# scverse/scanpy

Measured on AMD Instinct MI355X. Metric: cells/sec through pca+neighbors+leiden, 1M x 2k CSR, higher is better.
Workload: dtype bf16x3

## Files before the change

### scanpy_amd/_kernels.py

```python
from __future__ import annotations

import ctypes as C

import torch

from . import _lib
from ._device import ptr, require_gpu, stream_ptr, workspace_pool

import os as _os

_POISON = _os.environ.get("SCAMD_POISON_WORKSPACE") == "1"
_GUARD = _os.environ.get("SCAMD_GUARD") == "1"
_GUARD_BYTES = 4096
_CANARY = 0xC5
_guards: list = []


def _guarded(nbytes: int, dev: torch.device, label: str) -> torch.Tensor:
    pay = (int(nbytes) + 255) // 256 * 256
    raw = torch.empty(pay + 2 * _GUARD_BYTES, dtype=torch.uint8, device=dev)
    raw[:_GUARD_BYTES] = _CANARY
    raw[_GUARD_BYTES + int(nbytes):] = _CANARY
    _guards.append((label, raw, int(nbytes)))
    return raw[_GUARD_BYTES:_GUARD_BYTES + int(nbytes)]
# ... 232 lines not shown
    dev = require_gpu()
    lib = _lib.load()
    gp = (g + 127) // 128 * 128
    gram = _empty((gp, gp), dtype=torch.int64, device=dev)
    colsum = _empty(gp, dtype=torch.int64, device=dev)
    ws, wsz = _ws(lib.scamd_csr_gram_workspace_bytes(n, g), dev)
    rc = lib.scamd_csr_gram_f32(ptr(indptr), ptr(indices), ptr(data), n, g, data.numel(), int(scale_bits), ptr(gram),
                                gp, ptr(colsum), None, ptr(ws), wsz, stream_ptr())
    _check(rc, "scamd_csr_gram_f32")
    return gram, colsum


def spmm(indptr, indices, data, n: int, g: int, b: torch.Tensor, shift: torch.Tensor | None = None) -> torch.Tensor:
    dev = require_gpu()
    b = b.to(torch.float32).contiguous()
    assert b.shape[0] == g
    l = b.shape[1]
    y = _empty((n, l), dtype=torch.float32, device=dev)
    if shift is not None:
        shift = shift.to(torch.float32).contiguous()
    _check(_lib.load().scamd_spmm_csr_f32(ptr(indptr), ptr(indices), ptr(data), n, g, ptr(b), l, ptr(shift),
                                              ptr(y), stream_ptr()), "scamd_spmm_csr_f32")
    return y


def spmm_f64acc(indptr, indices, data, n_rows: int, b: torch.Tensor, scale: torch.Tensor | None = None,
                colsum: torch.Tensor | None = None) -> torch.Tensor:
    dev = require_gpu()
    lib = _lib.load()
    assert b.dtype == torch.float32 and b.is_contiguous()
    l = b.shape[1]
    nnz = data.numel()
    w = _empty((n_rows, l), dtype=torch.float64, device=dev)
    ws, wsz = _ws(lib.scamd_spmm_f64acc_workspace_bytes(n_rows, nnz, l), dev)
    rc = lib.scamd_spmm_csr_f32_f64acc(ptr(indptr), ptr(indices), ptr(data), n_rows, nnz, ptr(b), l, ptr(scale),
                                       ptr(colsum), ptr(w), ptr(ws), wsz, stream_ptr())
    _check(rc, "scamd_spmm_csr_f32_f64acc")
    return w


def dense_debug(op: int, in0: torch.Tensor, in1: torch.Tensor | None = None):
    dev = require_gpu()
    lib = _lib.load()
    in0 = in0.to(torch.float64).contiguous()
    flag = C.c_int(0)
    if op == 1:
        in1 = in1.to(torch.float64).contiguous()
        kdim, m = in0.shape
        n = in1.shape[1]
        out = _empty((m, n), dtype=torch.float64, device=dev)
        rc = lib.scamd_dense_debug_f64(1, ptr(in0), ptr(in1), m, n, kdim, ptr(out), None, C.byref(flag), stream_ptr())
        _check(rc, "scamd_dense_debug_f64")
        return out
    m = in0.shape[0]
    out0 = _empty((m, m) if op == 2 else (m,), dtype=torch.float64, device=dev)
    out1 = _empty((m, m), dtype=torch.float64, device=dev)
    rc = lib.scamd_dense_debug_f64(op, ptr(in0), None, m, m, m, ptr(out0), ptr(out1), C.byref(flag), stream_ptr())
    _check(rc, "scamd_dense_debug_f64")
    return (out0, int(flag.value)) if op == 2 else (out0, out1, int(flag.value))


def eigh_topk(a: torch.Tensor, k: int, *, seed: int = 0, tol: float = 2e-8):
    dev = require_gpu()
    lib = _lib.load()
    assert a.dtype == torch.float64 and a.dim() == 2 and a.shape[0] == a.shape[1] and a.is_cuda
    a = a.contiguous()
    g = a.shape[0]
    lam = _empty(k, dtype=torch.float64, device=dev)
    v = _empty((g, k), dtype=torch.float64, device=dev)
    info = (C.c_int32 * 12)()
    need = lib.scamd_eigh_topk_workspace_bytes(g, k)
    ws, wsz = _ws(need, dev)
    rc = lib.scamd_eigh_topk_f64(ptr(a), g, a.stride(0), k, int(seed) & (2**64 - 1), float(tol), ptr(lam), ptr(v), info,
                                 ptr(ws), wsz, stream_ptr())
    _check(rc, "scamd_eigh_topk_f64")
    resid = C.cast(C.byref(info, 16), C.POINTER(C.c_double))[0]
    return lam, v, {"n_outer": info[0], "n_gemm": info[1], "block_size": info[2], "chol_retries": info[3], "residual": resid}


def pca_csr(indptr, indices, data, n: int, g: int, n_comps: int, *, zero_center: bool = True, seed: int = 0,
            tol: float = 2e-8):
    dev = require_gpu()
    lib = _lib.load()
    k = int(n_comps)
    scores = _empty((n, k), dtype=torch.float32, device=dev)
    comps = _empty((k, g), dtype=torch.float64, device=dev)
    var = _empty(k, dtype=torch.float64, device=dev)
    ratio = _empty(k, dtype=torch.float64, device=dev)
    mean = _empty(g, dtype=torch.float64, device=dev)
    info = (C.c_int32 * 12)()
    need = lib.scamd_pca_csr_workspace_bytes(n, g, k)
    ws, wsz = _ws(need, dev)
    rc = lib.scamd_pca_csr_f32(ptr(indptr), ptr(indices), ptr(data), n, g, data.numel(), k, 1 if zero_center else 0,
                               int(seed) & (2**64 - 1), float(tol), ptr(scores), ptr(comps), ptr(var), ptr(ratio), ptr(mean),
                               info, ptr(ws), wsz, stream_ptr())
    _check(rc, "scamd_pca_csr_f32")
    resid = C.cast(C.byref(info, 16), C.POINTER(C.c_double))[0]
    return scores, comps, var, ratio, mean, {"n_outer": info[0], "n_gemm": info[1], "block_size": info[2],
                                             "chol_retries": info[3], "residual": resid, "scale_bits": info[6]}


def pca_solve_gram(gram_q: torch.Tensor, colsum_q: torch.Tensor, n_total: int, g: int, scale_bits: int, n_comps: int, *,
                   zero_center: bool = True, seed: int = 0, tol: float = 2e-8):
    dev = require_gpu()
    lib = _lib.load()
    k = int(n_comps)
# ... 249 lines not shown
```

### scanpy_amd/csrc/dense.hip

```cpp
#include "common.h"

#include <algorithm>
#include <cmath>
#include <cstdlib>
#include <vector>

namespace scamd {

using f64x4 = __attribute__((ext_vector_type(4))) double;

constexpr int DB_MAX = 128;
constexpr int DB_LD = DB_MAX + 2;
constexpr int DENSE_BATCH_HOST = DB_MAX - 32;

__device__ __forceinline__ unsigned int dhash32(unsigned int x) {
  x ^= x >> 16;
  x *= 0x7feb352dU;
  x ^= x >> 15;
  x *= 0x846ca68bU;
  x ^= x >> 16;
  return x;
}

template <int CTRL>
__device__ __forceinline__ double dpp_f64(double x) {
  const long long b = __double_as_longlong(x);
  const int lo = __builtin_amdgcn_update_dpp(0, (int)(b & 0xffffffffll), CTRL, 0xf, 0xf, false);
  const int hi = __builtin_amdgcn_update_dpp(0, (int)(b >> 32), CTRL, 0xf, 0xf, false);
  return __longlong_as_double(((long long)hi << 32) | (unsigned int)lo);
}
__device__ __forceinline__ double row16_sum(double x) {
  x += dpp_f64<0x128>(x);
  x += dpp_f64<0x124>(x);
  x += dpp_f64<0x122>(x);
  x += dpp_f64<0x121>(x);
  return x;
}
__device__ __forceinline__ double oct_sum(double x) {
  x += dpp_f64<0xB1>(x);
  x += dpp_f64<0x4E>(x);
  x += dpp_f64<0x141>(x);
  return x;
}

__global__ __launch_bounds__(512) void dgemm_tn_kernel(const double* __restrict__ P, int64_t ldp,
                                                       const double* __restrict__ Q, int64_t ldq, int M, int N, int K,
                                                       double alpha, const double* __restrict__ D1, int64_t ldd1,
                                                       double beta1, const double* __restrict__ D2, int64_t ldd2,
                                                       double beta2, double* __restrict__ C, int64_t ldc) {
  __shared__ double red[8][32 * 32];
  const int lane = threadIdx.x & 63, wave = threadIdx.x >> 6;
  const int l15 = lane & 15, kq = lane >> 4;
  const int m0 = blockIdx.x * 32, n0 = blockIdx.y * 32;
  const int kc = ((K + 7) / 8 + 3) / 4 * 4;
  const int kb = wave * kc, ke = min(K, kb + kc);
  f64x4 acc[2][2];
#pragma unroll
  for (int a = 0; a < 2; ++a)
#pragma unroll
    for (int b = 0; b < 2; ++b)
#pragma unroll
      for (int v = 0; v < 4; ++v) acc[a][b][v] = 0.0;
  const bool mv0 = m0 + l15 < M, mv1 = m0 + 16 + l15 < M;
  const bool nv0 = n0 + l15 < N, nv1 = n0 + 16 + l15 < N;
  const double* pp = P + m0 + l15;
  const double* qq = Q + n0 + l15;
#pragma unroll 4
  for (int k0 = kb; k0 < ke; k0 += 4) {
    const int kk = k0 + kq;
    const bool kv = kk < ke;
    const double a0 = (kv && mv0) ? pp[(int64_t)kk * ldp] : 0.0;
    const double a1 = (kv && mv1) ? pp[(int64_t)kk * ldp + 16] : 0.0;
    const double b0 = (kv && nv0) ? qq[(int64_t)kk * ldq] : 0.0;
    const double b1 = (kv && nv1) ? qq[(int64_t)kk * ldq + 16] : 0.0;
    acc[0][0] = __builtin_amdgcn_mfma_f64_16x16x4f64(a0, b0, acc[0][0], 0, 0, 0);
    acc[0][1] = __builtin_amdgcn_mfma_f64_16x16x4f64(a0, b1, acc[0][1], 0, 0, 0);
    acc[1][0] = __builtin_amdgcn_mfma_f64_16x16x4f64(a1, b0, acc[1][0], 0, 0, 0);
    acc[1][1] = __builtin_amdgcn_mfma_f64_16x16x4f64(a1, b1, acc[1][1], 0, 0, 0);
  }
#pragma unroll
  for (int a = 0; a < 2; ++a)
#pragma unroll
    for (int b = 0; b < 2; ++b)
#pragma unroll
      for (int v = 0; v < 4; ++v) red[wave][(16 * a + kq + 4 * v) * 32 + 16 * b + l15] = acc[a][b][v];
  __syncthreads();
#pragma unroll
  for (int j = 0; j < 2; ++j) {
    const int idx = threadIdx.x + 512 * j;
    const int r = idx >> 5, c = idx & 31;
    const int m = m0 + r, n = n0 + c;
    if (m < M && n < N) {
      double s = (((red[0][idx] + red[1][idx]) + (red[2][idx] + red[3][idx])) +
                  ((red[4][idx] + red[5][idx]) + (red[6][idx] + red[7][idx])));
      s *= alpha;
      if (D1) s += beta1 * D1[(int64_t)m * ldd1 + n];
      if (D2) s += beta2 * D2[(int64_t)m * ldd2 + n];
      C[(int64_t)m * ldc + n] = s;
    }
  }
}

static int dgemm_tn(hipStream_t s, const double* P, int64_t ldp, const double* Q, int64_t ldq, int M, int N, int K,
                    double alpha, const double* D1, int64_t ldd1, double beta1, const double* D2, int64_t ldd2,
                    double beta2, double* C, int64_t ldc) {
  hipLaunchKernelGGL(dgemm_tn_kernel, dim3((M + 31) / 32, (N + 31) / 32), dim3(512), 0, s, P, ldp, Q, ldq, M, N, K,
                     alpha, D1, ldd1, beta1, D2, ldd2, beta2, C, ldc);
  SCAMD_LAUNCH_CHECK();
  return SCAMD_OK;
}

__global__ __launch_bounds__(1024) void chol_factor_kernel(const double* __restrict__ G, int b, double shift,
                                                           double* __restrict__ S, int* __restrict__ flag) {
  extern __shared__ __attribute__((aligned(16))) double sm[];
  double* L = sm;
  double* dinv = sm + DB_MAX * DB_LD;
  const int tid = threadIdx.x;
  const int row = tid >> 3, part = tid & 7;
  for (int j = tid; j < b; j += 1024) {
    const double d = G[(int64_t)j * b + j];
    dinv[j] = d > 0.0 ? 1.0 / sqrt(d) : 0.0;
  }
  __syncthreads();
  for (int e = tid; e < b * b; e += 1024) {
    const int i = e / b, j = e - i * b;
    double v = G[(int64_t)i * b + j] * dinv[i] * dinv[j];
    if (i == j) v = (dinv[i] > 0.0 ? 1.0 : 0.0) + shift;
    L[i * DB_LD + j] = v;
  }
  __syncthreads();
  bool bad = false;
  __shared__ double sh_piv[2];
  for (int j = 0; j < b; ++j) {
    double acc = 0.0;
    const bool mine = row >= j && row < b;
    if (mine)
      for (int k = part; k < j; k += 8) acc = fma(L[row * DB_LD + k], L[j * DB_LD + k], acc);
    acc = oct_sum(acc);
    const double v = mine ? L[row * DB_LD + j] - acc : 0.0;
    if (row == j && part == 0) sh_piv[j & 1] = v;
    __syncthreads();
    const double piv = sh_piv[j & 1];
    if (!(piv > 0.0)) {
      bad = true;
      break;
    }
    if (mine && part == 0) L[row * DB_LD + j] = (row == j) ? sqrt(piv) : v / sqrt(piv);
    __syncthreads();
  }
  if (tid == 0) *flag = bad ? 1 : 0;
  if (bad) return;
  {
    const int c = row;
    const double xcc = c < b ? 1.0 / L[c * DB_LD + c] : 0.0;
    for (int j = 1; j < b; ++j) {
      double acc = 0.0;
      if (c < j) {
        for (int k = c + 1 + part; k < j; k += 8) acc = fma(L[j * DB_LD + k], L[c * DB_LD + k], acc);
        if (part == 0) acc = fma(L[j * DB_LD + c], xcc, acc);
      }
      acc = oct_sum(acc);
      if (c < j && part == 0) L[c * DB_LD + j] = -acc / L[j * DB_LD + j];
      __syncthreads();
    }
  }
  for (int e = tid; e < b * b; e += 1024) {
    const int k = e / b, n = e - k * b;
    double v = 0.0;
    if (n == k) v = 1.0 / L[k * DB_LD + k];
    else if (n > k) v = L[k * DB_LD + n];
    S[e] = v * dinv[k];
  }
}

__global__ __launch_bounds__(256) void panel_small_kernel(const double* __restrict__ Z, const double* __restrict__ S, int g,
                                                          int b, int bo , double* __restrict__ C) {
  __shared__ double zrow[8][DB_MAX];
  const int r = threadIdx.x >> 5, cq = threadIdx.x & 31;
  const int m = blockIdx.x * 8 + r;
  for (int k = cq; k < b; k += 32) zrow[r][k] = (m < g) ? Z[(int64_t)m * b + k] : 0.0;
  __syncthreads();
  if (m >= g) return;
  for (int n0 = cq * 4; n0 < bo; n0 += 128) {
    double c0 = 0.0, c1 = 0.0, c2 = 0.0, c3 = 0.0;
    for (int k = 0; k < b; ++k) {
      const double z = zrow[r][k];
      const double* sp = S + (int64_t)k * bo + n0;
      c0 = fma(z, sp[0], c0);
      if (n0 + 1 < bo) c1 = fma(z, sp[1], c1);
      if (n0 + 2 < bo) c2 = fma(z, sp[2], c2);
      if (n0 + 3 < bo) c3 = fma(z, sp[3], c3);
    }
    double* cp = C + (int64_t)m * bo + n0;
    cp[0] = c0;
    if (n0 + 1 < bo) cp[1] = c1;
    if (n0 + 2 < bo) cp[2] = c2;
    if (n0 + 3 < bo) cp[3] = c3;
  }
}

__global__ __launch_bounds__(512) void jacobi_eigh_kernel(const double* __restrict__ T, int b, double* __restrict__ theta,
                                                          double* __restrict__ Y, int* __restrict__ sweeps_out) {
  extern __shared__ __attribute__((aligned(16))) double sm[];
  double* W = sm;
  double* nrm = sm + DB_MAX * DB_LD;
  __shared__ float off_arr[64];
  __shared__ int rank_of[DB_MAX];
  const int tid = threadIdx.x;
  const int n2 = (b + 1) & ~1;
  for (int e = tid; e < n2 * DB_LD; e += 512) {
    const int c = e / DB_LD, i = e - c * DB_LD;
    W[e] = (c < b && i < b) ? T[(int64_t)i * b + c] : 0.0;
  }
  __syncthreads();
  const int grp = tid >> 3, t8 = tid & 7;
  const int nm1 = n2 - 1;
  int sweep = 0;
  for (; sweep < 30; ++sweep) {
    float my_off = 0.f;
    int p = grp == 0 ? nm1 : grp % nm1;
    int q = grp == 0 ? 0 : (nm1 - grp % nm1) % nm1;
    for (int step = 0; step < nm1; ++step) {
      const bool act = grp < n2 / 2 && p < b && q < b;
      if (act) {
        double* wp = W + p * DB_LD;
        double* wq = W + q * DB_LD;
        double a = 0.0, bb = 0.0, c = 0.0;
        for (int i = t8; i < b; i += 8) {
          const double x = wp[i], y = wq[i];
          a = fma(x, x, a);
          bb = fma(y, y, bb);
          c = fma(x, y, c);
        }
        a = oct_sum(a);
        bb = oct_sum(bb);
        c = oct_sum(c);
        const double ab = a * bb;
        if (c * c > 1e-30 * ab) {
          const double d = bb - a, tau = 2.0 * c;
          const double inv_r = rsqrt(fma(d, d, tau * tau));
          const double h = fma(0.5 * fabs(d), inv_r, 0.5);
          const double inv_cs = rsqrt(h);
          const double cs = h * inv_cs;
          const double sn = (d >= 0.0 ? 0.5 : -0.5) * tau * inv_r * inv_cs;
          for (int i = t8; i < b; i += 8) {
            const double x = wp[i], y = wq[i];
            wp[i] = cs * x - sn * y;
            wq[i] = sn * x + cs * y;
          }
          my_off = fmaxf(my_off, (float)(fabs(c) * rsqrt(ab)));
        }
      }
      if (grp != 0) {
        p = p + 1 == nm1 ? 0 : p + 1;
        q = q + 1 == nm1 ? 0 : q + 1;
      } else {
        q = step + 1;
      }
      __syncthreads();
    }
    if (t8 == 0) off_arr[grp] = my_off;
    __syncthreads();
    float off = 0.f;
    for (int i = 0; i < 64; ++i) off = fmaxf(off, off_arr[i]);
    __syncthreads();
    if (off < 1e-8f) {
      ++sweep;
      break;
    }
  }
  if (tid < n2) {
    double a = 0.0;
    for (int i = 0; i < b; ++i) a = fma(W[tid * DB_LD + i], W[tid * DB_LD + i], a);
    nrm[tid] = tid < b ? sqrt(a) : -1.0;
  }
  __syncthreads();
  if (tid < b) {
    int r = 0;
    const double me = nrm[tid];
    for (int j = 0; j < b; ++j) r += (nrm[j] > me || (nrm[j] == me && j < tid)) ? 1 : 0;
    rank_of[tid] = r;
  }
  __syncthreads();
  for (int c = grp; c < b; c += 64) {
    const double nv = nrm[c];
    const double inv = nv > 0.0 ? 1.0 / nv : 0.0;
    const int r = rank_of[c];
    if (t8 == 0) theta[r] = nv;
    for (int i = t8; i < b; i += 8) Y[(int64_t)i * b + r] = W[c * DB_LD + i] * inv;
  }
  if (tid == 0 && sweeps_out) *sweeps_out = sweep;
}

__global__ void randn_kernel(double* __restrict__ z, int64_t count, unsigned int seed) {
  const int64_t i = (int64_t)blockIdx.x * blockDim.x + threadIdx.x;
  if (i >= count) return;
  const unsigned int h1 = dhash32((unsigned int)i * 0x9E3779B1u + seed);
  const unsigned int h2 = dhash32(h1 ^ 0x85EBCA77u ^ (unsigned int)(i >> 32));
  const double u1 = ((double)h1 + 0.5) * (1.0 / 4294967296.0), u2 = ((double)h2 + 0.5) * (1.0 / 4294967296.0);
  z[i] = sqrt(-2.0 * log(u1)) * cos(6.283185307179586 * u2);
}

__global__ void axpby_kernel(int64_t count, double a, const double* __restrict__ x1, double b,
                             const double* __restrict__ x2, double* __restrict__ y) {
  const int64_t i = (int64_t)blockIdx.x * blockDim.x + threadIdx.x;
  if (i < count) y[i] = a * x1[i] + b * x2[i];
}

__global__ void symmetrize_kernel(double* __restrict__ t, int b) {
  const int e = blockIdx.x * blockDim.x + threadIdx.x;
  if (e >= b * b) return;
  const int i = e / b, j = e - i * b;
  if (j > i) {
    const double v = 0.5 * (t[(int64_t)i * b + j] + t[(int64_t)j * b + i]);
    t[(int64_t)i * b + j] = v;
    t[(int64_t)j * b + i] = v;
  }
}

__global__ __launch_bounds__(1024) void rq_minmax_kernel(const double* __restrict__ Z, const double* __restrict__ AZ, int g,
                                                         int b, double* __restrict__ out) {
  __shared__ double part[8][DB_MAX];
  const int c = threadIdx.x & 127, rr = threadIdx.x >> 7;
  double s = 0.0;
  if (c < b) {
    double s1 = 0.0, s2 = 0.0, s3 = 0.0;
    int m = rr;
    for (; m + 24 < g; m += 32) {
      s = fma(Z[(int64_t)m * b + c], AZ[(int64_t)m * b + c], s);
      s1 = fma(Z[(int64_t)(m + 8) * b + c], AZ[(int64_t)(m + 8) * b + c], s1);
      s2 = fma(Z[(int64_t)(m + 16) * b + c], AZ[(int64_t)(m + 16) * b + c], s2);
      s3 = fma(Z[(int64_t)(m + 24) * b + c], AZ[(int64_t)(m + 24) * b + c], s3);
    }
    for (; m < g; m += 8) s = fma(Z[(int64_t)m * b + c], AZ[(int64_t)m * b + c], s);
    s = (s + s1) + (s2 + s3);
  }
  part[rr][c] = s;
  __syncthreads();
  if (threadIdx.x == 0) {
    double mn = INFINITY, mx = -INFINITY;
    for (int j = 0; j < b; ++j) {
      double t = 0.0;
      for (int r = 0; r < 8; ++r) t += part[r][j];
      mn = fmin(mn, t);
      mx = fmax(mx, t);
    }
    out[1] = mn;
    out[2] = mx;
  }
}

__global__ __launch_bounds__(1024) void residual_kernel(const double* __restrict__ V, const double* __restrict__ AV,
                                                        const double* __restrict__ theta, int g, int b, int k,
                                                        double* __restrict__ out) {
  __shared__ double part[8][DB_MAX];
  const int c = threadIdx.x & 127, rr = threadIdx.x >> 7;
  double s = 0.0;
  if (c < k) {
    const double th = theta[c];
    double s1 = 0.0, s2 = 0.0, s3 = 0.0;
    int m = rr;
    for (; m + 24 < g; m += 32) {
      const double d0 = AV[(int64_t)m * b + c] - th * V[(int64_t)m * b + c];
      const double d1 = AV[(int64_t)(m + 8) * b + c] - th * V[(int64_t)(m + 8) * b + c];
      const double d2 = AV[(int64_t)(m + 16) * b + c] - th * V[(int64_t)(m + 16) * b + c];
      const double d3 = AV[(int64_t)(m + 24) * b + c] - th * V[(int64_t)(m + 24) * b + c];
      s = fma(d0, d0, s);
      s1 = fma(d1, d1, s1);
      s2 = fma(d2, d2, s2);
      s3 = fma(d3, d3, s3);
// ... 247 lines not shown
}

}

using namespace scamd;

extern "C" size_t scamd_eigh_topk_workspace_bytes(int64_t g, int k) {
  if (g < 1 || k < 1) return 0;
  Workspace ws(nullptr, 0);
  DenseBuffers d;
  dense_carve(ws, g, dense_block_size(g, k), &d);
  return ws.used();
}

extern "C" int scamd_eigh_topk_f64(const double* a, int64_t g, int64_t lda, int k, uint64_t seed, double tol,
                                   double* lam, double* v, int32_t* info_host, void* workspace, size_t workspace_bytes,
                                   scamd_stream_t stream) {
  SCAMD_REQUIRE(a && lam && v, SCAMD_EINVAL, "eigh_topk: null pointer");
  SCAMD_REQUIRE(g >= 1 && lda >= g && k >= 1 && k <= g, SCAMD_EINVAL, "eigh_topk: bad shape g=%lld k=%d", (long long)g, k);
  SCAMD_REQUIRE(g < ((int64_t)1 << 30), SCAMD_EUNSUPPORTED, "eigh_topk: g too large");
  const int b = dense_block_size(g, k);
  SCAMD_REQUIRE(b == g || k + 32 <= b, SCAMD_EUNSUPPORTED,
                "eigh_topk: k=%d needs a block beyond %d columns (use a full eigendecomposition)", k, DB_MAX);
  SCAMD_REQUIRE(b == g || g >= 2 * b, SCAMD_EUNSUPPORTED, "eigh_topk: g=%lld between %d and %d is served by a full eigh",
                (long long)g, DB_MAX, 2 * DB_MAX);
  DenseOp cx;
  cx.s = stream;
  cx.a = a;
  cx.lda = lda;
  cx.g = (int)g;
  Workspace ws(workspace, workspace_bytes);
  cx.carve(ws, b);
  SCAMD_REQUIRE(workspace && ws.ok, SCAMD_EWORKSPACE, "eigh_topk: workspace %zu < required %zu", workspace_bytes, ws.used());
  DenseStats st;
  int rc = dense_topk(cx, k, eigensolver_seed(seed, 12345u), tol, st);
  if (rc != SCAMD_OK) return rc;
  SCAMD_HIP_CHECK(hipMemcpyAsync(lam, cx.w.theta, sizeof(double) * k, hipMemcpyDeviceToDevice, stream));
  SCAMD_HIP_CHECK(hipMemcpy2DAsync(v, sizeof(double) * k, cx.d.z[3], sizeof(double) * b, sizeof(double) * k, (size_t)g,
                                   hipMemcpyDeviceToDevice, stream));
  SCAMD_HIP_CHECK(hipStreamSynchronize(stream));
  st.n_gemm = cx.n_gemm;
  st.n_chol_retry = cx.n_chol_retry;
  pack_dense_info(info_host, st, -1);
  return SCAMD_OK;
}

extern "C" int scamd_dense_debug_f64(int op, const double* in0, const double* in1, int m, int n, int kdim, double* out0,
                                     double* out1, int32_t* flag_host, scamd_stream_t stream) {
  SCAMD_REQUIRE(in0 && out0, SCAMD_EINVAL, "dense_debug: null pointer");
  if (op == 1) {
    SCAMD_REQUIRE(in1, SCAMD_EINVAL, "dense_debug: null pointer");
    int rc = dgemm_tn(stream, in0, m, in1, n, m, n, kdim, 1.0, nullptr, 0, 0.0, nullptr, 0, 0.0, out0, n);
    if (rc != SCAMD_OK) return rc;
  } else if (op == 2 || op == 3) {
    const int b = m;
    SCAMD_REQUIRE(b >= 1 && b <= DB_MAX, SCAMD_EINVAL, "dense_debug: b=%d", b);
    int* dflag = nullptr;
    SCAMD_HIP_CHECK(hipMalloc(reinterpret_cast<void**>(&dflag), 2 * sizeof(int)));
    SCAMD_HIP_CHECK(hipMemsetAsync(dflag, 0, 2 * sizeof(int), stream));
    int rc = prepare_lds_kernels();
    if (rc != SCAMD_OK) return rc;
    if (op == 2) {
      hipLaunchKernelGGL(chol_factor_kernel, dim3(1), dim3(1024), CHOL_LDS, stream, in0, b, 0.0, out0, dflag);
    } else {
      SCAMD_REQUIRE(out1, SCAMD_EINVAL, "dense_debug: null pointer");
      hipLaunchKernelGGL(jacobi_eigh_kernel, dim3(1), dim3(512), JAC_LDS, stream, in0, b, out0, out1, dflag + 1);
    }
    SCAMD_LAUNCH_CHECK();
    int h[2] = {0, 0};
    SCAMD_HIP_CHECK(hipMemcpyAsync(h, dflag, 2 * sizeof(int), hipMemcpyDeviceToHost, stream));
    SCAMD_HIP_CHECK(hipStreamSynchronize(stream));
    SCAMD_HIP_CHECK(hipFree(dflag));
    if (flag_host) *flag_host = op == 2 ? h[0] : h[1];
    return SCAMD_OK;
  } else {
    SCAMD_REQUIRE(false, SCAMD_EINVAL, "dense_debug: op=%d", op);
  }
  SCAMD_HIP_CHECK(hipStreamSynchronize(stream));
  return SCAMD_OK;
}

namespace scamd {
struct PcaBuffers {
  long long* gram; long long* colsum; float* v32; float* shift;
  void* gram_ws; size_t gram_ws_bytes; void* solve_ws; size_t solve_ws_bytes;
};
__global__ __launch_bounds__(256) void sum_kernel(const double* __restrict__ x, int g, double* __restrict__ out) {
  __shared__ double part[256];
  double s = 0.0;
  for (int i = threadIdx.x; i < g; i += 256) s += x[i];
  part[threadIdx.x] = s;
  __syncthreads();
  for (int o = 128; o > 0; o >>= 1) {
    if ((int)threadIdx.x < o) part[threadIdx.x] += part[threadIdx.x + o];
    __syncthreads();
  }
  if (threadIdx.x == 0) out[0] = part[0];
}
__global__ void variance_kernel(const double* __restrict__ theta, int k, double denom, const double* __restrict__ proj,
                                const double* __restrict__ varsum, double total_scale, double* __restrict__ variance,
                                double* __restrict__ ratio) {
  const int c = blockIdx.x * blockDim.x + threadIdx.x;
  if (c >= k) return;
  double ev = fmax(theta[c], 0.0) / denom;
  if (proj) ev = fmax(ev - proj[c] * proj[c], 0.0);
  variance[c] = ev;
  const double tot = varsum[0] * total_scale;
  ratio[c] = tot > 0.0 ? ev / tot : 0.0;
}
}

namespace scamd {
struct PcaSolveBuffers {
  double* a; double* var; double* varsum; double* proj; double* theta_all; double* deflate; void* dense_ws; size_t dense_ws_bytes;
};
static void pca_solve_carve(Workspace& ws, int64_t g, int k, PcaSolveBuffers* b) {
  b->a = ws.take<double>((size_t)g * g);
  b->var = ws.take<double>((size_t)g);
  b->varsum = ws.take<double>(8);
  b->proj = ws.take<double>((size_t)k + 8);
  b->theta_all = ws.take<double>((size_t)k + 8);
  b->deflate = ws.take<double>(k > DENSE_BATCH_HOST ? (size_t)DENSE_BATCH_HOST * g : 8);
  b->dense_ws_bytes = scamd_eigh_topk_workspace_bytes(g, std::min(k, DENSE_BATCH_HOST));
  b->dense_ws = ws.take<char>(b->dense_ws_bytes);
}
__global__ void copy_theta_kernel(const double* __restrict__ theta, int k, double* __restrict__ out) {
  const int c = blockIdx.x * blockDim.x + threadIdx.x;
// ... 457 lines not shown
```

### scanpy_amd/csrc/subspace.h

```cpp
#pragma once

namespace scamd {

struct SubspaceScratch {
  double* gm; double* smat; double* tmat; double* ymat;
  double* theta;
  int* flags;
};

static constexpr size_t CHOL_LDS = (size_t)(DB_MAX * DB_LD + DB_MAX) * sizeof(double);
static constexpr size_t JAC_LDS = (size_t)(DB_MAX * DB_LD + DB_MAX) * sizeof(double);

static int prepare_lds_kernels() {
  SCAMD_HIP_CHECK(hipFuncSetAttribute(reinterpret_cast<const void*>(chol_factor_kernel),
                                      hipFuncAttributeMaxDynamicSharedMemorySize, (int)CHOL_LDS));
  SCAMD_HIP_CHECK(hipFuncSetAttribute(reinterpret_cast<const void*>(jacobi_eigh_kernel),
                                      hipFuncAttributeMaxDynamicSharedMemorySize, (int)JAC_LDS));
  return SCAMD_OK;
}

static unsigned int eigensolver_seed(uint64_t seed, unsigned int salt) {
  return (unsigned int)(seed ^ (seed >> 32)) * 0x9E3779B1u + salt;
}

template <class Op>
static int panel_times_small(Op& op, const double* z, const double* small, double* out) {
  hipLaunchKernelGGL(panel_small_kernel, dim3((unsigned)((op.rows() + 7) / 8)), dim3(256), 0, op.s, z, small, (int)op.rows(), op.b,
                     op.b, out);
  SCAMD_LAUNCH_CHECK();
  return SCAMD_OK;
}

template <class Op>
static int cholqr2(Op& op, double* zin, double* tmp, double* zout, bool filtered, int plain_rounds) {
  const int b = op.b;
  double* cur = zin;
  double* other = tmp;
  int plain_ok = 0, shifted_rounds = 0;
  const double s0 = 11.0 * ((double)op.rows() * b + (double)b * (b + 1)) * 2.220446049250313e-16 * b;
  while (plain_ok < plain_rounds) {
    int rc = op.gram(cur, b, cur, b, op.w.gm);
    if (rc != SCAMD_OK) return rc;
    double shift = (filtered && plain_ok == 0 && shifted_rounds == 0) ? s0 : 0.0;
    for (int attempt = shift > 0.0 ? 1 : 0;; ++attempt) {
      int bad = 0;
      hipLaunchKernelGGL(chol_factor_kernel, dim3(1), dim3(1024), CHOL_LDS, op.s, op.w.gm, b, shift, op.w.smat, op.w.flags);
      SCAMD_LAUNCH_CHECK();
      SCAMD_READBACK_NOW(&bad, op.w.flags, sizeof(int), op.s);
      if (!bad) break;
      SCAMD_REQUIRE(attempt < 4 && shifted_rounds < 8, SCAMD_EUNSUPPORTED,
                    "%s: CholeskyQR gave up on the block (%d shifted rounds, attempt %d)", op.who, shifted_rounds, attempt);
      shift = shift == 0.0 ? s0 : shift * 1e3;
      ++op.n_chol_retry;
    }
    const bool was_shifted = shift > 0.0;
    double* dst = (!was_shifted && plain_ok == plain_rounds - 1) ? zout : other;
    rc = panel_times_small(op, cur, op.w.smat, dst);
    if (rc != SCAMD_OK) return rc;
    if (dst == other) std::swap(cur, other);
    if (was_shifted) {
      plain_ok = 0;
      ++shifted_rounds;
    } else {
      ++plain_ok;
    }
  }
  return SCAMD_OK;
}

template <class Op>
static int rayleigh_ritz(Op& op, const double* z, double* az, double* v, double* av, double* h_theta) {
  const int b = op.b;
  int rc = op.apply(z, nullptr, 1.0, 0.0, 0.0, az);
  if (rc != SCAMD_OK) return rc;
  rc = op.gram(z, b, az, b, op.w.tmat);
  if (rc != SCAMD_OK) return rc;
  hipLaunchKernelGGL(symmetrize_kernel, dim3((b * b + 255) / 256), dim3(256), 0, op.s, op.w.tmat, b);
  SCAMD_LAUNCH_CHECK();
  hipLaunchKernelGGL(jacobi_eigh_kernel, dim3(1), dim3(512), JAC_LDS, op.s, op.w.tmat, b, op.w.theta, op.w.ymat, op.w.flags + 1);
  SCAMD_LAUNCH_CHECK();
  rc = panel_times_small(op, z, op.w.ymat, v);
  if (rc != SCAMD_OK) return rc;
  rc = panel_times_small(op, az, op.w.ymat, av);
  if (rc != SCAMD_OK) return rc;
  SCAMD_READBACK(h_theta, op.w.theta, sizeof(double) * b, op.s);
  return SCAMD_OK;
}

static int chebyshev_degree(double c, double top, double theta_k, int max_degree) {
  const double e = 0.5 * c, center = 0.5 * c;
  const double x1 = (top - center) / e, xk = std::max((theta_k - center) / e, 1.0);
  const double spread = std::acosh(x1) - std::acosh(xk);
  return spread > 0.0 ? std::max(4, std::min(max_degree, (int)std::floor(20.7 / spread))) : max_degree;
}

template <class Op>
static int chebyshev_filter(Op& op, const double* vv, const double* avv, double c, double top, int m, double* y0, double* y1, double* z,
                            double** result) {
  const int64_t cnt = op.rows() * op.b;
  const double e = 0.5 * c, center = 0.5 * c;
  double sigma = e / (top - center);
  const double sigma1 = sigma;
  hipLaunchKernelGGL(axpby_kernel, dim3((unsigned)((cnt + 255) / 256)), dim3(256), 0, op.s, cnt, sigma1 / e, avv, -center * sigma1 / e,
                     vv, y0);
  SCAMD_LAUNCH_CHECK();
  const double* yprev = vv;
  double* ycur = y0;
  double* ynew = y1;
  for (int it = 2; it <= m; ++it) {
    const double sigma2 = 1.0 / (2.0 / sigma1 - sigma);
    const int rc = op.apply(ycur, yprev, 2.0 * sigma2 / e, center, sigma * sigma2, ynew);
    if (rc != SCAMD_OK) return rc;
    double* old = (yprev == vv) ? z : const_cast<double*>(yprev);
    yprev = ycur;
    ycur = ynew;
    ynew = old;
    sigma = sigma2;
  }
  *result = ycur;
  return SCAMD_OK;
}

}
```

Before: 21.72 million.

## Rework dense subspace kernels: prefetched GEMM, LDS panel product, fused symmetrize

The gram GEMM now software-pipelines register batches of K-slices with clamped loads, so per-step bounds checks leave the load path. The panel-times-small kernel stages both Z rows and the small matrix in LDS, and one launch now covers both the z and az products. Symmetrization is folded into the Jacobi eigensolver load, and the Jacobi and Cholesky inner loops are unrolled with templated widths. This trims launches and global traffic in the Rayleigh-Ritz and CholeskyQR steps, at the cost of more registers, larger dynamic LDS and much more code to get right.

```diff
diff --git a/scanpy_amd/_kernels.py b/scanpy_amd/_kernels.py
--- a/scanpy_amd/_kernels.py
+++ b/scanpy_amd/_kernels.py
@@ -308,6 +308,22 @@
         rc = lib.scamd_dense_debug_f64(1, ptr(in0), ptr(in1), m, n, kdim, ptr(out), None, C.byref(flag), stream_ptr())
         _check(rc, "scamd_dense_debug_f64")
         return out
+    if op == 4:
+        in1 = in1.to(torch.float64).contiguous()
+        m, kdim = in0.shape
+        n = in1.shape[1]
+        out = _empty((m, n), dtype=torch.float64, device=dev)
+        rc = lib.scamd_dense_debug_f64(4, ptr(in0), ptr(in1), m, n, kdim, ptr(out), None, C.byref(flag), stream_ptr())
+        _check(rc, "scamd_dense_debug_f64")
+        return out
+    if op == 5:
+        in1 = in1.to(torch.float64).contiguous()
+        m, kdim = in0.shape[0] // 2, in0.shape[1]
+        n = in1.shape[1]
+        out0, out1 = (_empty((m, n), dtype=torch.float64, device=dev) for _ in range(2))
+        rc = lib.scamd_dense_debug_f64(5, ptr(in0), ptr(in1), m, n, kdim, ptr(out0), ptr(out1), C.byref(flag), stream_ptr())
+        _check(rc, "scamd_dense_debug_f64")
+        return out0, out1
     m = in0.shape[0]
     out0 = _empty((m, m) if op == 2 else (m,), dtype=torch.float64, device=dev)
     out1 = _empty((m, m), dtype=torch.float64, device=dev)
diff --git a/scanpy_amd/csrc/dense.hip b/scanpy_amd/csrc/dense.hip
--- a/scanpy_amd/csrc/dense.hip
+++ b/scanpy_amd/csrc/dense.hip
@@ -12,6 +12,7 @@
 constexpr int DB_MAX = 128;
 constexpr int DB_LD = DB_MAX + 2;
 constexpr int DENSE_BATCH_HOST = DB_MAX - 32;
+constexpr int GEMM_KB = 8;
 
 __device__ __forceinline__ unsigned int dhash32(unsigned int x) {
   x ^= x >> 16;
@@ -63,20 +64,58 @@
       for (int v = 0; v < 4; ++v) acc[a][b][v] = 0.0;
   const bool mv0 = m0 + l15 < M, mv1 = m0 + 16 + l15 < M;
   const bool nv0 = n0 + l15 < N, nv1 = n0 + 16 + l15 < N;
-  const double* pp = P + m0 + l15;
-  const double* qq = Q + n0 + l15;
-#pragma unroll 4
-  for (int k0 = kb; k0 < ke; k0 += 4) {
-    const int kk = k0 + kq;
-    const bool kv = kk < ke;
-    const double a0 = (kv && mv0) ? pp[(int64_t)kk * ldp] : 0.0;
-    const double a1 = (kv && mv1) ? pp[(int64_t)kk * ldp + 16] : 0.0;
-    const double b0 = (kv && nv0) ? qq[(int64_t)kk * ldq] : 0.0;
-    const double b1 = (kv && nv1) ? qq[(int64_t)kk * ldq + 16] : 0.0;
-    acc[0][0] = __builtin_amdgcn_mfma_f64_16x16x4f64(a0, b0, acc[0][0], 0, 0, 0);
-    acc[0][1] = __builtin_amdgcn_mfma_f64_16x16x4f64(a0, b1, acc[0][1], 0, 0, 0);
-    acc[1][0] = __builtin_amdgcn_mfma_f64_16x16x4f64(a1, b0, acc[1][0], 0, 0, 0);
-    acc[1][1] = __builtin_amdgcn_mfma_f64_16x16x4f64(a1, b1, acc[1][1], 0, 0, 0);
+  const double* pp0 = P + min(m0 + l15, M - 1);
+  const double* pp1 = P + min(m0 + 16 + l15, M - 1);
+  const double* qq0 = Q + min(n0 + l15, N - 1);
+  const double* qq1 = Q + min(n0 + 16 + l15, N - 1);
+  const int nsteps = ke > kb ? (ke - kb + 3) >> 2 : 0;
+  double ca0[GEMM_KB], ca1[GEMM_KB], cb0[GEMM_KB], cb1[GEMM_KB];
+  double na0[GEMM_KB], na1[GEMM_KB], nb0[GEMM_KB], nb1[GEMM_KB];
+  if (nsteps > 0) {
+#pragma unroll
+    for (int j = 0; j < GEMM_KB; ++j) {
+      const int64_t kk = min(kb + 4 * j + kq, K - 1);
+      ca0[j] = pp0[kk * ldp];
+      ca1[j] = pp1[kk * ldp];
+      cb0[j] = qq0[kk * ldq];
+      cb1[j] = qq1[kk * ldq];
+    }
+  }
+  for (int s0 = 0; s0 < nsteps; s0 += GEMM_KB) {
+    const bool more = s0 + GEMM_KB < nsteps;
+    if (more) {
+#pragma unroll
+      for (int j = 0; j < GEMM_KB; ++j) {
+        const int64_t kk = min(kb + 4 * (s0 + GEMM_KB + j) + kq, K - 1);
+        na0[j] = pp0[kk * ldp];
+        na1[j] = pp1[kk * ldp];
+        nb0[j] = qq0[kk * ldq];
+        nb1[j] = qq1[kk * ldq];
+      }
+    }
+#pragma unroll
+    for (int j = 0; j < GEMM_KB; ++j) {
+      if (s0 + j < nsteps) {
+        const bool kv = kb + 4 * (s0 + j) + kq < ke;
+        const double a0 = (kv && mv0) ? ca0[j] : 0.0;
+        const double a1 = (kv && mv1) ? ca1[j] : 0.0;
+        const double b0 = (kv && nv0) ? cb0[j] : 0.0;
+        const double b1 = (kv && nv1) ? cb1[j] : 0.0;
+        acc[0][0] = __builtin_amdgcn_mfma_f64_16x16x4f64(a0, b0, acc[0][0], 0, 0, 0);
+        acc[0][1] = __builtin_amdgcn_mfma_f64_16x16x4f64(a0, b1, acc[0][1], 0, 0, 0);
+        acc[1][0] = __builtin_amdgcn_mfma_f64_16x16x4f64(a1, b0, acc[1][0], 0, 0, 0);
+        acc[1][1] = __builtin_amdgcn_mfma_f64_16x16x4f64(a1, b1, acc[1][1], 0, 0, 0);
+      }
+    }
+    if (more) {
+#pragma unroll
+      for (int j = 0; j < GEMM_KB; ++j) {
+        ca0[j] = na0[j];
+        ca1[j] = na1[j];
+        cb0[j] = nb0[j];
+        cb1[j] = nb1[j];
+      }
+    }
   }
 #pragma unroll
   for (int a = 0; a < 2; ++a)
@@ -130,22 +169,42 @@
   }
   __syncthreads();
   bool bad = false;
-  __shared__ double sh_piv[2];
+  __shared__ double sh_piv[2], sh_root[2];
   for (int j = 0; j < b; ++j) {
     double acc = 0.0;
     const bool mine = row >= j && row < b;
-    if (mine)
-      for (int k = part; k < j; k += 8) acc = fma(L[row * DB_LD + k], L[j * DB_LD + k], acc);
+    double ljj = 0.0;
+    if (mine) {
+      const double* lr = L + row * DB_LD;
+      const double* lj = L + j * DB_LD;
+      ljj = lr[j];
+      for (int k0 = part; k0 < j; k0 += 32) {
+        double x[4], y[4];
+#pragma unroll
+        for (int t = 0; t < 4; ++t) {
+          const int kk = min(k0 + 8 * t, j - 1);
+          x[t] = lr[kk];
+          y[t] = lj[kk];
+        }
+#pragma unroll
+        for (int t = 0; t < 4; ++t)
+          if (k0 + 8 * t < j) acc = fma(x[t], y[t], acc);
+      }
+    }
     acc = oct_sum(acc);
-    const double v = mine ? L[row * DB_LD + j] - acc : 0.0;
-    if (row == j && part == 0) sh_piv[j & 1] = v;
+    const double v = mine ? ljj - acc : 0.0;
+    if (row == j && part == 0) {
+      sh_piv[j & 1] = v;
+      sh_root[j & 1] = sqrt(v);
+    }
     __syncthreads();
     const double piv = sh_piv[j & 1];
     if (!(piv > 0.0)) {
       bad = true;
       break;
     }
-    if (mine && part == 0) L[row * DB_LD + j] = (row == j) ? sqrt(piv) : v / sqrt(piv);
+    const double root = sh_root[j & 1];
+    if (mine && part == 0) L[row * DB_LD + j] = (row == j) ? root : v / root;
     __syncthreads();
   }
   if (tid == 0) *flag = bad ? 1 : 0;
@@ -154,13 +213,28 @@
     const int c = row;
     const double xcc = c < b ? 1.0 / L[c * DB_LD + c] : 0.0;
     for (int j = 1; j < b; ++j) {
-      double acc = 0.0;
+      double acc = 0.0, pivot = 1.0;
       if (c < j) {
-        for (int k = c + 1 + part; k < j; k += 8) acc = fma(L[j * DB_LD + k], L[c * DB_LD + k], acc);
-        if (part == 0) acc = fma(L[j * DB_LD + c], xcc, acc);
+        const double* lj = L + j * DB_LD;
+        const double* lc = L + c * DB_LD;
+        const double ljc = lj[c], ljj = lj[j];
+        for (int k0 = c + 1 + part; k0 < j; k0 += 32) {
+          double x[4], y[4];
+#pragma unroll
+          for (int t = 0; t < 4; ++t) {
+            const int kk = min(k0 + 8 * t, j - 1);
+            x[t] = lj[kk];
+            y[t] = lc[kk];
+          }
+#pragma unroll
+          for (int t = 0; t < 4; ++t)
+            if (k0 + 8 * t < j) acc = fma(x[t], y[t], acc);
+        }
+        if (part == 0) acc = fma(ljc, xcc, acc);
+        pivot = ljj;
       }
       acc = oct_sum(acc);
-      if (c < j && part == 0) L[c * DB_LD + j] = -acc / L[j * DB_LD + j];
+      if (c < j && part == 0) L[c * DB_LD + j] = -acc / pivot;
       __syncthreads();
     }
   }
@@ -173,48 +247,95 @@
   }
 }
 
-__global__ __launch_bounds__(256) void panel_small_kernel(const double* __restrict__ Z, const double* __restrict__ S, int g,
-                                                          int b, int bo , double* __restrict__ C) {
-  __shared__ double zrow[8][DB_MAX];
-  const int r = threadIdx.x >> 5, cq = threadIdx.x & 31;
-  const int m = blockIdx.x * 8 + r;
-  for (int k = cq; k < b; k += 32) zrow[r][k] = (m < g) ? Z[(int64_t)m * b + k] : 0.0;
+constexpr int PANEL_SB = 8;
+constexpr int panel_lds_doubles(int b, int cq_shift) {
+  return b * (4 << cq_shift) + 2 * (256 >> cq_shift) * (b | 1);
+}
+__global__ __launch_bounds__(256) void panel_small_kernel(const double* __restrict__ Z0, const double* __restrict__ Z1,
+                                                          const double* __restrict__ S, int g, int b, int bo, int cq_shift,
+                                                          double* __restrict__ C0, double* __restrict__ C1) {
+  extern __shared__ __attribute__((aligned(16))) double sm[];
+  const int tid = threadIdx.x;
+  const int W = 4 << cq_shift, rpp = 256 >> cq_shift, rows = 2 * rpp;
+  const int zld = b | 1;
+  double* Ss = sm;
+  double* Zs = sm + b * W;
+  const double* __restrict__ Z = blockIdx.y ? Z1 : Z0;
+  double* __restrict__ C = blockIdx.y ? C1 : C0;
+  const int m0 = blockIdx.x * rows;
+  {
+    double zv[8];
+    const int zcount = rows * b;
+    const int64_t zlast = (int64_t)g * b - 1;
+#pragma unroll
+    for (int u = 0; u < 8; ++u) zv[u] = Z[min((int64_t)m0 * b + tid + 256 * u, zlast)];
+    const int scount = b * W;
+    const int wmask = W - 1, wshift = cq_shift + 2;
+    double cur[PANEL_SB], nxt[PANEL_SB];
+#pragma unroll
+    for (int u = 0; u < PANEL_SB; ++u) {
+      const int e = tid + 256 * u;
+      cur[u] = S[min(e >> wshift, b - 1) * bo + min(e & wmask, bo - 1)];
+    }
+#pragma unroll
+    for (int u = 0; u < 8; ++u) {
+      const int e = tid + 256 * u;
+      if (e < zcount) {
+        const int r = e / b;
+        Zs[r * zld + (e - r * b)] = (m0 + r < g) ? zv[u] : 0.0;
+      }
+    }
+    for (int e0 = 0; e0 < scount; e0 += 256 * PANEL_SB) {
+      const bool more = e0 + 256 * PANEL_SB < scount;
+      if (more) {
+#pragma unroll
+        for (int u = 0; u < PANEL_SB; ++u) {
+          const int e = e0 + 256 * PANEL_SB + tid + 256 * u;
+          nxt[u] = S[min(e >> wshift, b - 1) * bo + min(e & wmask, bo - 1)];
+        }
+      }
+#pragma unroll
+      for (int u = 0; u < PANEL_SB; ++u) {
+        const int e = e0 + tid + 256 * u;
+        if (e < scount) Ss[e] = ((e & wmask) < bo) ? cur[u] : 0.0;
+      }
+      if (more) {
+#pragma unroll
+        for (int u = 0; u < PANEL_SB; ++u) cur[u] = nxt[u];
+      }
+    }
+  }
   __syncthreads();
-  if (m >= g) return;
-  for (int n0 = cq * 4; n0 < bo; n0 += 128) {
-    double c0 = 0.0, c1 = 0.0, c2 = 0.0, c3 = 0.0;
-    for (int k = 0; k < b; ++k) {
-      const double z = zrow[r][k];
-      const double* sp = S + (int64_t)k * bo + n0;
-      c0 = fma(z, sp[0], c0);
-      if (n0 + 1 < bo) c1 = fma(z, sp[1], c1);
-      if (n0 + 2 < bo) c2 = fma(z, sp[2], c2);
-      if (n0 + 3 < bo) c3 = fma(z, sp[3], c3);
-    }
-    double* cp = C + (int64_t)m * bo + n0;
-    cp[0] = c0;
-    if (n0 + 1 < bo) cp[1] = c1;
-    if (n0 + 2 < bo) cp[2] = c2;
-    if (n0 + 3 < bo) cp[3] = c3;
-  }
-}
-
-__global__ __launch_bounds__(512) void jacobi_eigh_kernel(const double* __restrict__ T, int b, double* __restrict__ theta,
-                                                          double* __restrict__ Y, int* __restrict__ sweeps_out) {
-  extern __shared__ __attribute__((aligned(16))) double sm[];
-  double* W = sm;
-  double* nrm = sm + DB_MAX * DB_LD;
-  __shared__ float off_arr[64];
-  __shared__ int rank_of[DB_MAX];
-  const int tid = threadIdx.x;
-  const int n2 = (b + 1) & ~1;
-  for (int e = tid; e < n2 * DB_LD; e += 512) {
-    const int c = e / DB_LD, i = e - c * DB_LD;
-    W[e] = (c < b && i < b) ? T[(int64_t)i * b + c] : 0.0;
-  }
-  __syncthreads();
+  const int cq = tid & ((1 << cq_shift) - 1), rg = tid >> cq_shift;
+  const double* sp = Ss + 4 * cq;
+  const double* z0 = Zs + rg * zld;
+  const double* z1 = Zs + (rg + rpp) * zld;
+  double c0[4] = {0.0, 0.0, 0.0, 0.0}, c1[4] = {0.0, 0.0, 0.0, 0.0};
+#pragma unroll 8
+  for (int k = 0; k < b; ++k) {
+    const double za = z0[k], zb = z1[k];
+#pragma unroll
+    for (int j = 0; j < 4; ++j) {
+      const double sv = sp[k * W + j];
+      c0[j] = fma(za, sv, c0[j]);
+      c1[j] = fma(zb, sv, c1[j]);
+    }
+  }
+  const int n0 = 4 * cq;
+#pragma unroll
+  for (int j = 0; j < 4; ++j) {
+    if (n0 + j < bo) {
+      if (m0 + rg < g) C[(int64_t)(m0 + rg) * bo + n0 + j] = c0[j];
+      if (m0 + rg + rpp < g) C[(int64_t)(m0 + rg + rpp) * bo + n0 + j] = c1[j];
+    }
+  }
+}
+
+template <int NJ>
+__device__ __forceinline__ int jacobi_sweeps(double* W, float* off_arr, int b, int n2, int tid) {
   const int grp = tid >> 3, t8 = tid & 7;
   const int nm1 = n2 - 1;
+  const bool last_in = t8 + 8 * (NJ - 1) < b;
   int sweep = 0;
   for (; sweep < 30; ++sweep) {
     float my_off = 0.f;
@@ -223,14 +344,22 @@
     for (int step = 0; step < nm1; ++step) {
       const bool act = grp < n2 / 2 && p < b && q < b;
       if (act) {
-        double* wp = W + p * DB_LD;
-        double* wq = W + q * DB_LD;
+        double* wp = W + p * DB_LD + t8;
+        double* wq = W + q * DB_LD + t8;
+        double x[NJ], y[NJ];
+#pragma unroll
+        for (int j = 0; j < NJ; ++j) {
+          x[j] = wp[8 * j];
+          y[j] = wq[8 * j];
+        }
         double a = 0.0, bb = 0.0, c = 0.0;
-        for (int i = t8; i < b; i += 8) {
-          const double x = wp[i], y = wq[i];
-          a = fma(x, x, a);
-          bb = fma(y, y, bb);
-          c = fma(x, y, c);
+#pragma unroll
+        for (int j = 0; j < NJ; ++j) {
+          if (j < NJ - 1 || last_in) {
+            a = fma(x[j], x[j], a);
+            bb = fma(y[j], y[j], bb);
+            c = fma(x[j], y[j], c);
+          }
         }
         a = oct_sum(a);
         bb = oct_sum(bb);
@@ -243,10 +372,12 @@
           const double inv_cs = rsqrt(h);
           const double cs = h * inv_cs;
           const double sn = (d >= 0.0 ? 0.5 : -0.5) * tau * inv_r * inv_cs;
-          for (int i = t8; i < b; i += 8) {
-            const double x = wp[i], y = wq[i];
-            wp[i] = cs * x - sn * y;
-            wq[i] = sn * x + cs * y;
+#pragma unroll
+          for (int j = 0; j < NJ; ++j) {
+            if (j < NJ - 1 || last_in) {
+              wp[8 * j] = cs * x[j] - sn * y[j];
+              wq[8 * j] = sn * x[j] + cs * y[j];
+            }
           }
           my_off = fmaxf(my_off, (float)(fabs(c) * rsqrt(ab)));
         }
@@ -269,8 +400,50 @@
       break;
     }
   }
+  return sweep;
+}
+
+__global__ __launch_bounds__(512) void jacobi_eigh_kernel(const double* __restrict__ T, int b, int symmetrize,
+                                                          double* __restrict__ theta, double* __restrict__ Y,
+                                                          int* __restrict__ sweeps_out) {
+  extern __shared__ __attribute__((aligned(16))) double sm[];
+  double* W = sm;
+  double* nrm = sm + DB_MAX * DB_LD;
+  __shared__ float off_arr[64];
+  __shared__ int rank_of[DB_MAX];
+  const int tid = threadIdx.x;
+  const int n2 = (b + 1) & ~1;
+  for (int e0 = tid; e0 < n2 * DB_LD; e0 += 512 * 4) {
+    double t1[4], t2[4];
+#pragma unroll
+    for (int u = 0; u < 4; ++u) {
+      const int e = e0 + 512 * u;
+      const int c = min(e / DB_LD, b - 1), i = min(e % DB_LD, b - 1);
+      t1[u] = T[(int64_t)i * b + c];
+      t2[u] = T[(int64_t)(symmetrize ? c : i) * b + (symmetrize ? i : c)];
+    }
+#pragma unroll
+    for (int u = 0; u < 4; ++u) {
+      const int e = e0 + 512 * u;
+      const int c = e / DB_LD, i = e - c * DB_LD;
+      if (e < n2 * DB_LD) W[e] = (c < b && i < b) ? ((symmetrize && i != c) ? 0.5 * (t1[u] + t2[u]) : t1[u]) : 0.0;
+    }
+  }
+  __syncthreads();
+  const int grp = tid >> 3, t8 = tid & 7;
+  int sweep = 0;
+  switch ((b + 7) >> 3) {
+#define SCAMD_JACOBI_CASE(NJ) case NJ: sweep = jacobi_sweeps<NJ>(W, off_arr, b, n2, tid); break;
+    SCAMD_JACOBI_CASE(1) SCAMD_JACOBI_CASE(2) SCAMD_JACOBI_CASE(3) SCAMD_JACOBI_CASE(4)
+    SCAMD_JACOBI_CASE(5) SCAMD_JACOBI_CASE(6) SCAMD_JACOBI_CASE(7) SCAMD_JACOBI_CASE(8)
+    SCAMD_JACOBI_CASE(9) SCAMD_JACOBI_CASE(10) SCAMD_JACOBI_CASE(11) SCAMD_JACOBI_CASE(12)
+    SCAMD_JACOBI_CASE(13) SCAMD_JACOBI_CASE(14) SCAMD_JACOBI_CASE(15) SCAMD_JACOBI_CASE(16)
+#undef SCAMD_JACOBI_CASE
+    default: break;
+  }
   if (tid < n2) {
     double a = 0.0;
+#pragma unroll 8
     for (int i = 0; i < b; ++i) a = fma(W[tid * DB_LD + i], W[tid * DB_LD + i], a);
     nrm[tid] = tid < b ? sqrt(a) : -1.0;
   }
@@ -305,17 +478,6 @@
                              const double* __restrict__ x2, double* __restrict__ y) {
   const int64_t i = (int64_t)blockIdx.x * blockDim.x + threadIdx.x;
   if (i < count) y[i] = a * x1[i] + b * x2[i];
-}
-
-__global__ void symmetrize_kernel(double* __restrict__ t, int b) {
-  const int e = blockIdx.x * blockDim.x + threadIdx.x;
-  if (e >= b * b) return;
-  const int i = e / b, j = e - i * b;
-  if (j > i) {
-    const double v = 0.5 * (t[(int64_t)i * b + j] + t[(int64_t)j * b + i]);
-    t[(int64_t)i * b + j] = v;
-    t[(int64_t)j * b + i] = v;
-  }
 }
 
 __global__ __launch_bounds__(1024) void rq_minmax_kernel(const double* __restrict__ Z, const double* __restrict__ AZ, int g,
@@ -669,7 +831,7 @@
     SCAMD_REQUIRE(in1, SCAMD_EINVAL, "dense_debug: null pointer");
     int rc = dgemm_tn(stream, in0, m, in1, n, m, n, kdim, 1.0, nullptr, 0, 0.0, nullptr, 0, 0.0, out0, n);
     if (rc != SCAMD_OK) return rc;
-  } else if (op == 2 || op == 3) {
+  } else if (op == 2 || op == 3 || op == 6) {
     const int b = m;
     SCAMD_REQUIRE(b >= 1 && b <= DB_MAX, SCAMD_EINVAL, "dense_debug: b=%d", b);
     int* dflag = nullptr;
@@ -681,7 +843,7 @@
       hipLaunchKernelGGL(chol_factor_kernel, dim3(1), dim3(1024), CHOL_LDS, stream, in0, b, 0.0, out0, dflag);
     } else {
       SCAMD_REQUIRE(out1, SCAMD_EINVAL, "dense_debug: null pointer");
-      hipLaunchKernelGGL(jacobi_eigh_kernel, dim3(1), dim3(512), JAC_LDS, stream, in0, b, out0, out1, dflag + 1);
+      hipLaunchKernelGGL(jacobi_eigh_kernel, dim3(1), dim3(512), JAC_LDS, stream, in0, b, op == 6 ? 1 : 0, out0, out1, dflag + 1);
     }
     SCAMD_LAUNCH_CHECK();
     int h[2] = {0, 0};
@@ -690,6 +852,12 @@
     SCAMD_HIP_CHECK(hipFree(dflag));
     if (flag_host) *flag_host = op == 2 ? h[0] : h[1];
     return SCAMD_OK;
+  } else if (op == 4 || op == 5) {
+    SCAMD_REQUIRE(in1 && (op == 4 || out1), SCAMD_EINVAL, "dense_debug: null pointer");
+    int rc = prepare_lds_kernels();
+    if (rc != SCAMD_OK) return rc;
+    rc = panel_small(stream, in0, op == 5 ? in0 + (int64_t)m * kdim : nullptr, in1, m, kdim, n, out0, op == 5 ? out1 : nullptr);
+    if (rc != SCAMD_OK) return rc;
   } else {
     SCAMD_REQUIRE(false, SCAMD_EINVAL, "dense_debug: op=%d", op);
   }
diff --git a/scanpy_amd/csrc/subspace.h b/scanpy_amd/csrc/subspace.h
--- a/scanpy_amd/csrc/subspace.h
+++ b/scanpy_amd/csrc/subspace.h
@@ -10,12 +10,15 @@
 
 static constexpr size_t CHOL_LDS = (size_t)(DB_MAX * DB_LD + DB_MAX) * sizeof(double);
 static constexpr size_t JAC_LDS = (size_t)(DB_MAX * DB_LD + DB_MAX) * sizeof(double);
+static constexpr size_t PANEL_LDS_MAX = (size_t)panel_lds_doubles(DB_MAX, 5) * sizeof(double);
 
 static int prepare_lds_kernels() {
   SCAMD_HIP_CHECK(hipFuncSetAttribute(reinterpret_cast<const void*>(chol_factor_kernel),
                                       hipFuncAttributeMaxDynamicSharedMemorySize, (int)CHOL_LDS));
   SCAMD_HIP_CHECK(hipFuncSetAttribute(reinterpret_cast<const void*>(jacobi_eigh_kernel),
                                       hipFuncAttributeMaxDynamicSharedMemorySize, (int)JAC_LDS));
+  SCAMD_HIP_CHECK(hipFuncSetAttribute(reinterpret_cast<const void*>(panel_small_kernel),
+                                      hipFuncAttributeMaxDynamicSharedMemorySize, (int)PANEL_LDS_MAX));
   return SCAMD_OK;
 }
 
@@ -23,12 +26,21 @@
   return (unsigned int)(seed ^ (seed >> 32)) * 0x9E3779B1u + salt;
 }
 
+static int panel_small(hipStream_t s, const double* z0, const double* z1, const double* small, int64_t rows, int b, int bo,
+                       double* c0, double* c1) {
+  int cq_shift = 0;
+  while ((4 << cq_shift) < bo) ++cq_shift;
+  SCAMD_REQUIRE(rows >= 1 && rows < ((int64_t)1 << 31) && b >= 1 && bo >= 1 && bo <= DB_MAX && b <= (4 << cq_shift), SCAMD_EINVAL,
+                "panel product: bad shape rows=%lld b=%d bo=%d", (long long)rows, b, bo);
+  const int rows_per = 2 * (256 >> cq_shift);
+  hipLaunchKernelGGL(panel_small_kernel, dim3((unsigned)((rows + rows_per - 1) / rows_per), z1 ? 2 : 1), dim3(256),
+                     (size_t)panel_lds_doubles(b, cq_shift) * sizeof(double), s, z0, z1, small, (int)rows, b, bo, cq_shift, c0, c1);
+  SCAMD_LAUNCH_CHECK();
+  return SCAMD_OK;
+}
 template <class Op>
 static int panel_times_small(Op& op, const double* z, const double* small, double* out) {
-  hipLaunchKernelGGL(panel_small_kernel, dim3((unsigned)((op.rows() + 7) / 8)), dim3(256), 0, op.s, z, small, (int)op.rows(), op.b,
-                     op.b, out);
-  SCAMD_LAUNCH_CHECK();
-  return SCAMD_OK;
+  return panel_small(op.s, z, nullptr, small, op.rows(), op.b, op.b, out, nullptr);
 }
 
 template <class Op>
@@ -75,13 +87,9 @@
   if (rc != SCAMD_OK) return rc;
   rc = op.gram(z, b, az, b, op.w.tmat);
   if (rc != SCAMD_OK) return rc;
-  hipLaunchKernelGGL(symmetrize_kernel, dim3((b * b + 255) / 256), dim3(256), 0, op.s, op.w.tmat, b);
+  hipLaunchKernelGGL(jacobi_eigh_kernel, dim3(1), dim3(512), JAC_LDS, op.s, op.w.tmat, b, 1, op.w.theta, op.w.ymat, op.w.flags + 1);
   SCAMD_LAUNCH_CHECK();
-  hipLaunchKernelGGL(jacobi_eigh_kernel, dim3(1), dim3(512), JAC_LDS, op.s, op.w.tmat, b, op.w.theta, op.w.ymat, op.w.flags + 1);
-  SCAMD_LAUNCH_CHECK();
-  rc = panel_times_small(op, z, op.w.ymat, v);
-  if (rc != SCAMD_OK) return rc;
-  rc = panel_times_small(op, az, op.w.ymat, av);
+  rc = panel_small(op.s, z, az, op.w.ymat, op.rows(), b, b, v, av);
   if (rc != SCAMD_OK) return rc;
   SCAMD_READBACK(h_theta, op.w.theta, sizeof(double) * b, op.s);
   return SCAMD_OK;
```

After: 22.15 million, median of 6. 2.0% higher.
